# JiawangBian/SC-SfMLearner-Release

Measured on AMD Instinct MI355X. Metric: train images/sec (+ warp-loss ms/step) KITTI 256x832 RN18, higher is better.
Workload: dtype f32; 1 GPU; configs[1]: kitti 256x832, batch 12/GPU, 2 refs (seq 3), ResNet18 DispNet + ResNet18 PoseNet, ssim+mask+auto-mask, zeros padding, 1 scale; global_batch=12, parallelism=1 GPU, memory_format=contiguous (NCHW)

## Files before the change

### __graft_entry__.py

```python
import os
import sys

ROOT = os.path.dirname(os.path.abspath(__file__))
PKG = os.path.join(ROOT, "sc-sfmlearner-release_amd")
for p in (ROOT, PKG):
    if p not in sys.path:
        sys.path.insert(0, p)


def build() -> None:
    from scsfm_hip import _lib, build as hip_build
    path = hip_build.build(force=False)
    lib = _lib.CLib(path)
    assert lib._dll.scsfm_abi_version() == _lib.ABI_VERSION
    nets_path = hip_build.build_nets(force=False)
    nets = _lib.CLib(nets_path, _lib.NETS_HEADER, _lib.NETS_ABI_VERSION, "scsfm_nets_")
    eval_path = hip_build.build_eval(force=False)
    ev = _lib.CLib(eval_path, _lib.EVAL_HEADER, _lib.EVAL_ABI_VERSION, "scsfm_eval_")
    odom_path = hip_build.build_odom(force=False)
    od = _lib.CLib(odom_path, _lib.ODOM_HEADER, _lib.ODOM_ABI_VERSION, "scsfm_odom_")
    import inverse_warp
    import loss_functions
    import models
    from scsfm_hip import decoder, depth_eval, odometry
    from oracle import scsfm_oracle
    print(f"[build] {path}: {len(lib.decls)} entry points resolved")
    print(f"[build] {nets_path}: {len(nets.decls)} entry points resolved")
    print(f"[build] {eval_path}: {len(ev.decls)} entry points resolved")
    print(f"[build] {odom_path}: {len(od.decls)} entry points resolved")


def smoke() -> None:
    import torch

    import loss_functions as LF
    from oracle import scsfm_oracle as O
    from scsfm_hip import _lib, synth

    assert torch.cuda.is_available(), "smoke() needs a HIP device"
    lib = _lib.get()
    assert lib.path.endswith("libscsfm_hip.so")
    dev = torch.device("cuda:0")
    d = synth.make_batch(2, 128, 416, n_ref=2, seed=0, depth="smooth")

    def leaves(device):
        mv = lambda t: t.to(device).clone().requires_grad_(True)
        return ([mv(t) for t in d["tgt_depth"]], [[mv(t) for t in r] for r in d["ref_depths"]],
                [mv(p) for p in d["poses"]], [mv(p) for p in d["poses_inv"]])

    td, rd, ps, pi = leaves(dev)
    tgt, refs, K = d["tgt_img"].to(dev), [r.to(dev) for r in d["ref_imgs"]], d["intrinsics"].to(dev)
    photo, geom = LF.compute_photo_and_geometry_loss(tgt, refs, K, td, rd, ps, pi, 1, 1, 1, 1, "zeros")
    smooth = LF.compute_smooth_loss(td, tgt, rd, refs)
    (photo + 0.1 * smooth + 0.5 * geom).backward()
    torch.cuda.synchronize()

    td_c, rd_c, ps_c, pi_c = leaves("cpu")
    photo_c, geom_c = O.photo_and_geometry_loss(d["tgt_img"], d["ref_imgs"], d["intrinsics"], td_c, rd_c, ps_c, pi_c,
                                                1, 1, 1, 1, "zeros")
    smooth_c = O.smooth_loss(td_c, d["tgt_img"], rd_c, d["ref_imgs"])
    (photo_c + 0.1 * smooth_c + 0.5 * geom_c).backward()
    for name, a, b in (("photo", photo, photo_c), ("geom", geom, geom_c), ("smooth", smooth, smooth_c)):
        err = abs(float(a) - float(b))
        print(f"[smoke] {name}: hip {float(a):.7f} oracle {float(b):.7f} |d| {err:.2e}")
        assert err <= 1e-5, name
    pairs = [("g_tgt_depth", td[0].grad, td_c[0].grad), ("g_ref0_depth", rd[0][0].grad, rd_c[0][0].grad),
             ("g_ref1_depth", rd[1][0].grad, rd_c[1][0].grad), ("g_pose0", ps[0].grad, ps_c[0].grad),
             ("g_pose_inv1", pi[1].grad, pi_c[1].grad)]
    for name, a, b in pairs:
        scale = float(b.abs().max())
        bad = ((a.cpu() - b).abs() > 0.01 * scale).double().mean().item()
        print(f"[smoke] {name}: scale {scale:.3e} share of entries off by >1% of scale {bad:.2e}")
        assert bad <= 2e-3, name
    print("[smoke] ok")


if __name__ == "__main__":
    build()
    if "--smoke" in sys.argv:
        smoke()
```

### sc-sfmlearner-release_amd/models/resnet_encoder.py

```python
from __future__ import absolute_import, division, print_function

import numpy as np
import torch
import torch.nn as nn


def _conv3x3(cin, cout, stride=1):
    return nn.Conv2d(cin, cout, kernel_size=3, stride=stride, padding=1, bias=False)


class BasicBlock(nn.Module):
    expansion = 1

    def __init__(self, inplanes, planes, stride=1, downsample=None):
        super().__init__()
        self.conv1 = _conv3x3(inplanes, planes, stride)
        self.bn1 = nn.BatchNorm2d(planes)
        self.relu = nn.ReLU(inplace=True)
        self.conv2 = _conv3x3(planes, planes)
        self.bn2 = nn.BatchNorm2d(planes)
        self.downsample = downsample

    def forward(self, x):
        identity = x if self.downsample is None else self.downsample(x)
        out = self.relu(self.bn1(self.conv1(x)))
        out = self.bn2(self.conv2(out))
        return self.relu(out + identity)


class Bottleneck(nn.Module):
    expansion = 4

    def __init__(self, inplanes, planes, stride=1, downsample=None):
        super().__init__()
        self.conv1 = nn.Conv2d(inplanes, planes, kernel_size=1, bias=False)
        self.bn1 = nn.BatchNorm2d(planes)
        self.conv2 = _conv3x3(planes, planes, stride)
        self.bn2 = nn.BatchNorm2d(planes)
        self.conv3 = nn.Conv2d(planes, planes * 4, kernel_size=1, bias=False)
        self.bn3 = nn.BatchNorm2d(planes * 4)
        self.relu = nn.ReLU(inplace=True)
        self.downsample = downsample

    def forward(self, x):
        identity = x if self.downsample is None else self.downsample(x)
        out = self.relu(self.bn1(self.conv1(x)))
        out = self.relu(self.bn2(self.conv2(out)))
        out = self.bn3(self.conv3(out))
        return self.relu(out + identity)


class ResNet(nn.Module):

    def __init__(self, block, layers, num_classes=1000, num_input_images=1):
        super().__init__()
        self.inplanes = 64
        self.conv1 = nn.Conv2d(num_input_images * 3, 64, kernel_size=7, stride=2, padding=3, bias=False)
        self.bn1 = nn.BatchNorm2d(64)
        self.relu = nn.ReLU(inplace=True)
        self.maxpool = nn.MaxPool2d(kernel_size=3, stride=2, padding=1)
        self.layer1 = self._make_layer(block, 64, layers[0])
        self.layer2 = self._make_layer(block, 128, layers[1], stride=2)
        self.layer3 = self._make_layer(block, 256, layers[2], stride=2)
        self.layer4 = self._make_layer(block, 512, layers[3], stride=2)
        self.avgpool = nn.AdaptiveAvgPool2d((1, 1))
        self.fc = nn.Linear(512 * block.expansion, num_classes)
        for m in self.modules():
            if isinstance(m, nn.Conv2d):
                nn.init.kaiming_normal_(m.weight, mode='fan_out', nonlinearity='relu')
            elif isinstance(m, nn.BatchNorm2d):
                nn.init.constant_(m.weight, 1)
                nn.init.constant_(m.bias, 0)

    def _make_layer(self, block, planes, blocks, stride=1):
        downsample = None
        if stride != 1 or self.inplanes != planes * block.expansion:
            downsample = nn.Sequential(
                nn.Conv2d(self.inplanes, planes * block.expansion, kernel_size=1, stride=stride, bias=False),
                nn.BatchNorm2d(planes * block.expansion))
        layers = [block(self.inplanes, planes, stride, downsample)]
        self.inplanes = planes * block.expansion
        layers += [block(self.inplanes, planes) for _ in range(1, blocks)]
        return nn.Sequential(*layers)


_CFG = {18: (BasicBlock, [2, 2, 2, 2]), 50: (Bottleneck, [3, 4, 6, 3])}


def imagenet_weights_path(num_layers):
    import os
    root = os.environ.get("SCSFM_IMAGENET_WEIGHTS")
    if not root:
        return None
    path = os.path.join(root, "resnet{}.pth".format(num_layers))
    return path if os.path.exists(path) else None


class ResnetEncoder(nn.Module):

    def __init__(self, num_layers, pretrained, num_input_images=1):
        super().__init__()
        if num_layers not in _CFG:
            raise ValueError("{} is not a valid number of resnet layers".format(num_layers))
        block, layers = _CFG[num_layers]
        self.num_ch_enc = np.array([64, 64, 128, 256, 512])
        if num_layers > 34:
            self.num_ch_enc[1:] *= 4
        self.encoder = ResNet(block, layers, num_input_images=num_input_images)
        if pretrained:
            path = imagenet_weights_path(num_layers)
            if path is None:
                raise RuntimeError("ImageNet-pretrained weights are not reachable offline: set SCSFM_IMAGENET_WEIGHTS "
                                   "to a directory holding resnet{}.pth, or use --with-pretrain 0".format(num_layers))
            loaded = torch.load(path, map_location="cpu")
            loaded['conv1.weight'] = torch.cat([loaded['conv1.weight']] * num_input_images, 1) / num_input_images
            self.encoder.load_state_dict(loaded)
        for p in self.encoder.fc.parameters():
            p.requires_grad_(False)

    def forward(self, input_image):
        e = self.encoder
        f0 = e.relu(e.bn1(e.conv1(input_image)))
        f1 = e.layer1(e.maxpool(f0))
        f2 = e.layer2(f1)
        f3 = e.layer3(f2)
        f4 = e.layer4(f3)
        self.features = [f0, f1, f2, f3, f4]
        return self.features
```

### sc-sfmlearner-release_amd/scsfm_hip/_lib.py

```python
from __future__ import annotations

import ctypes
import os
import re
import threading

import torch

HERE = os.path.dirname(os.path.abspath(__file__))
HEADER = os.path.join(os.path.dirname(os.path.dirname(HERE)), "include", "scsfm_hip.h")
LIB_PATH = os.environ.get("SCSFM_HIP_LIB") or os.path.join(HERE, "libscsfm_hip.so")

ABI_VERSION = 9

_CTYPES = {"int": ctypes.c_int, "unsigned": ctypes.c_uint, "size_t": ctypes.c_size_t, "double": ctypes.c_double}
_DECL = re.compile(r"^(int|size_t)\s+(scsfm_\w+)\s*\(([^)]*)\)\s*;", re.M | re.S)


def parse_header(path=HEADER):
    text = open(path).read()
    text = re.sub(r"/\*.*?\*/", "", text, flags=re.S)
    out = {}
    for ret, name, args in _DECL.findall(text):
        argtypes = []
        args = " ".join(args.split())
        if args and args != "void":
            for a in args.split(","):
                a = a.strip()
                if "*" in a:
                    argtypes.append(ctypes.c_void_p)
                else:
                    argtypes.append(_CTYPES[a.split()[0]])
        out[name] = (_CTYPES[ret], argtypes)
    return out


class ScsfmError(RuntimeError):
    pass


class CLib:

    def __init__(self, path, header=HEADER, abi=ABI_VERSION, prefix="scsfm_"):
        self.path = path
        self._dll = ctypes.CDLL(path)
        self.decls = parse_header(header)
        self._fn = {}
        self._prefix = prefix
        for name, (ret, argtypes) in self.decls.items():
            try:
                fn = getattr(self._dll, name)
            except AttributeError as e:
                raise ScsfmError(f"{path} does not export {name} (declared in {header})") from e
            fn.restype = ret
            fn.argtypes = argtypes
            self._fn[name] = fn
        if self._fn[prefix + "abi_version"]() != abi:
            raise ScsfmError(f"{path}: ABI version mismatch")

    def source_id(self):
        buf = ctypes.create_string_buffer(64)
        self._fn[self._prefix + "source_id"](buf, 64)
        return buf.value.decode()

    def call(self, name, *args):
        rc = self._fn[name](*args)
        if rc != 0:
            kind = "rejected argument" if rc == -1 else "hipError_t"
            raise ScsfmError(f"{name} failed with status {rc} ({kind})")

    def size(self, name, *args):
        return int(self._fn[name](*args))


_lock = threading.Lock()
_lib = None


def get() -> CLib:
    global _lib
    if _lib is None:
        with _lock:
            if _lib is None:
                from . import build as _build
                own = "SCSFM_HIP_LIB" not in os.environ
                if own and _build.is_stale():
                    have = _build.binary_source_id(LIB_PATH)
                    try:
                        _build.build()
                    except Exception as e:
                        what = f"was built from other sources ({have}) than the tree's ({_build.source_id()})" if have \
                            else "is missing (or carries no source id)"
                        raise ScsfmError(f"{LIB_PATH} {what} and cannot be built here: {e}") from e
                lib = CLib(LIB_PATH)
                if own and lib.source_id() != _build.source_id():
                    raise ScsfmError(f"{LIB_PATH}: its source id {lib.source_id()} is not the tree's {_build.source_id()}")
                _lib = lib
    return _lib


NETS_HEADER = os.path.join(os.path.dirname(os.path.dirname(HERE)), "include", "scsfm_nets.h")
NETS_LIB_PATH = os.path.join(HERE, "libscsfm_nets.so")
NETS_ABI_VERSION = 1
_nets = None


def get_nets() -> CLib:
    global _nets
    if _nets is None:
        with _lock:
            if _nets is None:
                from . import build as _build
                if _build.nets_is_stale():
                    have = _build.binary_source_id(NETS_LIB_PATH)
                    try:
                        _build.build_nets()
                    except Exception as e:
                        raise ScsfmError(f"{NETS_LIB_PATH} is stale or missing ({have}) and cannot be built here: {e}") \
                            from e
                lib = CLib(NETS_LIB_PATH, NETS_HEADER, NETS_ABI_VERSION, "scsfm_nets_")
                if lib.source_id() != _build.nets_source_id():
                    raise ScsfmError(f"{NETS_LIB_PATH}: its source id {lib.source_id()} is not the tree's "
                                     f"{_build.nets_source_id()}")
                _nets = lib
    return _nets


EVAL_HEADER = os.path.join(os.path.dirname(os.path.dirname(HERE)), "include", "scsfm_eval.h")
EVAL_LIB_PATH = os.path.join(HERE, "libscsfm_eval.so")
EVAL_ABI_VERSION = 1
_eval = None


def get_eval() -> CLib:
    global _eval
    if _eval is None:
        with _lock:
            if _eval is None:
                from . import build as _build
                if _build.eval_is_stale():
                    have = _build.binary_source_id(EVAL_LIB_PATH)
                    try:
                        _build.build_eval()
                    except Exception as e:
                        raise ScsfmError(f"{EVAL_LIB_PATH} is stale or missing ({have}) and cannot be built here: {e}") \
                            from e
                lib = CLib(EVAL_LIB_PATH, EVAL_HEADER, EVAL_ABI_VERSION, "scsfm_eval_")
                if lib.source_id() != _build.eval_source_id():
                    raise ScsfmError(f"{EVAL_LIB_PATH}: its source id {lib.source_id()} is not the tree's "
                                     f"{_build.eval_source_id()}")
                _eval = lib
    return _eval


ODOM_HEADER = os.path.join(os.path.dirname(os.path.dirname(HERE)), "include", "scsfm_odom.h")
ODOM_LIB_PATH = os.path.join(HERE, "libscsfm_odom.so")
ODOM_ABI_VERSION = 1
_odom = None


def get_odom() -> CLib:
    global _odom
    if _odom is None:
        with _lock:
            if _odom is None:
                from . import build as _build
                if _build.odom_is_stale():
                    have = _build.binary_source_id(ODOM_LIB_PATH)
                    try:
                        _build.build_odom()
                    except Exception as e:
                        raise ScsfmError(f"{ODOM_LIB_PATH} is stale or missing ({have}) and cannot be built here: {e}") \
                            from e
                lib = CLib(ODOM_LIB_PATH, ODOM_HEADER, ODOM_ABI_VERSION, "scsfm_odom_")
                if lib.source_id() != _build.odom_source_id():
                    raise ScsfmError(f"{ODOM_LIB_PATH}: its source id {lib.source_id()} is not the tree's "
                                     f"{_build.odom_source_id()}")
                _odom = lib
    return _odom
```

### sc-sfmlearner-release_amd/scsfm_hip/build.py

```python
from __future__ import annotations

import contextlib
import fcntl
import glob
import hashlib
import os
import shutil
import subprocess
import sys
import tempfile

HERE = os.path.dirname(os.path.abspath(__file__))
CSRC = os.path.join(os.path.dirname(HERE), "csrc")
LIB = os.path.join(HERE, "libscsfm_hip.so")
LOCK = LIB + ".lock"
LOG = LIB + ".buildlog"
INCLUDE = os.path.join(os.path.dirname(os.path.dirname(HERE)), "include")
NETS_CSRC = os.path.join(os.path.dirname(HERE), "csrc_nets")
NETS_LIB = os.path.join(HERE, "libscsfm_nets.so")
EVAL_CSRC = os.path.join(os.path.dirname(HERE), "csrc_eval")
EVAL_LIB = os.path.join(HERE, "libscsfm_eval.so")
ODOM_CSRC = os.path.join(os.path.dirname(HERE), "csrc_odom")
ODOM_LIB = os.path.join(HERE, "libscsfm_odom.so")
ARCH = "gfx950"
FLAGS = ["-O3", "-std=c++17", "-fPIC", "-shared", f"--offload-arch={ARCH}", "-munsafe-fp-atomics",
         "-fno-gpu-rdc", "-Wall", "-Wno-unused-function",
         "-fno-slp-vectorize"]
ID_MARKER = b"scsfm-source-id:"


def sources():
    return sorted(glob.glob(os.path.join(CSRC, "*.hip")))


def deps():
    return sources() + sorted(glob.glob(os.path.join(CSRC, "*.h"))) + \
        [os.path.join(INCLUDE, "scsfm_hip.h")]


def nets_sources():
    return sorted(glob.glob(os.path.join(NETS_CSRC, "*.hip")))


def nets_deps():
    return nets_sources() + sorted(glob.glob(os.path.join(NETS_CSRC, "*.h"))) + [os.path.join(INCLUDE, "scsfm_nets.h")]


def eval_sources():
    return sorted(glob.glob(os.path.join(EVAL_CSRC, "*.hip")))


def eval_deps():
    return eval_sources() + sorted(glob.glob(os.path.join(EVAL_CSRC, "*.h"))) + [os.path.join(INCLUDE, "scsfm_eval.h")]


def odom_sources():
    return sorted(glob.glob(os.path.join(ODOM_CSRC, "*.hip")))


def odom_deps():
    return odom_sources() + sorted(glob.glob(os.path.join(ODOM_CSRC, "*.h"))) + [os.path.join(INCLUDE, "scsfm_odom.h")]


def _hash(files, extra=()):
    h = hashlib.sha256()
    for path in files:
        h.update(os.path.basename(path).encode())
        h.update(open(path, "rb").read())
    h.update(" ".join(FLAGS).encode())
    if extra:
        h.update(b"\0extra:" + " ".join(extra).encode())
    return h.hexdigest()[:16]


def source_id(extra=()):
    files = deps()
    if any("SCSFM_WITH_MARCH" in e or "variants" in e for e in extra):
        vsrc = os.path.join(os.path.dirname(os.path.dirname(HERE)), "variants", "src")
        files = files + sorted(p for p in glob.glob(os.path.join(vsrc, "*")) if os.path.isfile(p))
    return _hash(files, extra)


def nets_source_id():
    return _hash(nets_deps())


def eval_source_id():
    return _hash(eval_deps())


def odom_source_id():
    return _hash(odom_deps())


def binary_source_id(path=LIB):
    try:
        blob = open(path, "rb").read()
    except OSError:
        return None
    i = blob.find(ID_MARKER)
    if i < 0:
        return None
    j = i + len(ID_MARKER)
    return blob[j:j + 16].decode("ascii", "replace")


def is_stale():
    return binary_source_id(LIB) != source_id()


def nets_is_stale():
    return binary_source_id(NETS_LIB) != nets_source_id()


def eval_is_stale():
    return binary_source_id(EVAL_LIB) != eval_source_id()


def odom_is_stale():
    return binary_source_id(ODOM_LIB) != odom_source_id()


@contextlib.contextmanager
def _build_lock(lock=None):
    fd = os.open(lock or LOCK, os.O_CREAT | os.O_RDWR, 0o644)
    try:
        fcntl.flock(fd, fcntl.LOCK_EX)
        yield
    finally:
        try:
            fcntl.flock(fd, fcntl.LOCK_UN)
        finally:
            os.close(fd)


def build(force=False, verbose=True, extra=()):
    extra = tuple(extra)
    return _build(LIB, source_id(extra), sources(), extra, force, verbose)


def build_nets(force=False, verbose=True):
    return _build(NETS_LIB, nets_source_id(), nets_sources(), ("-I", INCLUDE), force, verbose)


def build_eval(force=False, verbose=True):
    return _build(EVAL_LIB, eval_source_id(), eval_sources(), ("-I", INCLUDE), force, verbose)


def build_odom(force=False, verbose=True):
    return _build(ODOM_LIB, odom_source_id(), odom_sources(), ("-I", INCLUDE), force, verbose)


def _build(lib, want, srcs, extra, force, verbose):
    if not force and binary_source_id(lib) == want:
        return lib
    with _build_lock(lib + ".lock"):
        if not force and binary_source_id(lib) == want:
            return lib
        hipcc = shutil.which("hipcc") or "/opt/rocm/bin/hipcc"
        name = os.path.basename(lib)
        if not os.path.exists(hipcc):
            raise RuntimeError(f"hipcc not found: {name} cannot be built on this machine")
        fd, tmp = tempfile.mkstemp(prefix=name[:-len(".so")] + ".", suffix=f".{os.getpid()}.tmp", dir=HERE)
        os.close(fd)
        try:
            cmd = [hipcc, *FLAGS, f'-DSCSFM_SOURCE_ID="{want}"', *extra, "-o", tmp, *srcs]
            if verbose:
                print("[scsfm_hip.build]", " ".join(cmd), flush=True)
            subprocess.run(cmd, check=True)
            os.chmod(tmp, 0o755)
            os.replace(tmp, lib)
            with open(lib + ".buildlog", "a") as f:
                f.write(f"{want} {os.getpid()}\n")
        finally:
            if os.path.exists(tmp):
                os.unlink(tmp)
    return lib


if __name__ == "__main__":
    build(force="--force" in sys.argv)
    build_nets(force="--force" in sys.argv)
    build_eval(force="--force" in sys.argv)
    build_odom(force="--force" in sys.argv)
    print(LIB)
    print(NETS_LIB)
    print(EVAL_LIB)
    print(ODOM_LIB)
```

Measured before the change: 125.2 images/s.

## Add fused HIP BatchNorm+ReLU+residual and maxpool kernels for ResNet encoder

Adds a new HIP library with training-mode BatchNorm kernels that fuse the normalisation with an optional ReLU and residual add. Statistics are reduced in double precision across split blocks per channel. It also adds a max-pool forward that stores a compact uint8 argmax, and a matching backward. Autograd wrappers expose these as `bn_act` and `max_pool`, with build and ABI plumbing for a separate shared library. The aim is to cut the separate elementwise kernel launches and memory passes of the stock BN, ReLU and add ops in ResNet18, at the cost of custom code that must match PyTorch BN semantics.

```diff
diff --git a/__graft_entry__.py b/__graft_entry__.py
--- a/__graft_entry__.py
+++ b/__graft_entry__.py
@@ -19,15 +19,18 @@
     ev = _lib.CLib(eval_path, _lib.EVAL_HEADER, _lib.EVAL_ABI_VERSION, "scsfm_eval_")
     odom_path = hip_build.build_odom(force=False)
     od = _lib.CLib(odom_path, _lib.ODOM_HEADER, _lib.ODOM_ABI_VERSION, "scsfm_odom_")
+    enc_path = hip_build.build_enc(force=False)
+    enc = _lib.CLib(enc_path, _lib.ENC_HEADER, _lib.ENC_ABI_VERSION, "scsfm_enc_")
     import inverse_warp
     import loss_functions
     import models
-    from scsfm_hip import decoder, depth_eval, odometry
+    from scsfm_hip import decoder, depth_eval, encoder, odometry
     from oracle import scsfm_oracle
     print(f"[build] {path}: {len(lib.decls)} entry points resolved")
     print(f"[build] {nets_path}: {len(nets.decls)} entry points resolved")
     print(f"[build] {eval_path}: {len(ev.decls)} entry points resolved")
     print(f"[build] {odom_path}: {len(od.decls)} entry points resolved")
+    print(f"[build] {enc_path}: {len(enc.decls)} entry points resolved")
 
 
 def smoke() -> None:
diff --git a/include/scsfm_enc.h b/include/scsfm_enc.h
--- /dev/null
+++ b/include/scsfm_enc.h
@@ -0,0 +1,32 @@
+#ifndef SCSFM_ENC_H_
+#define SCSFM_ENC_H_
+
+#include <stddef.h>
+
+#ifdef __cplusplus
+extern "C" {
+#endif
+
+int scsfm_enc_abi_version(void);
+int scsfm_enc_source_id(char* buf, size_t n);
+
+size_t scsfm_enc_bn_workspace_bytes(int B, int C, int H, int W);
+
+int scsfm_enc_bn_fwd_f32(int B, int C, int H, int W, int mode, double eps, double momentum, const float* x,
+                         const float* identity, const float* gamma, const float* beta, float* y, float* stat,
+                         float* running_mean, float* running_var, long long* num_batches_tracked, void* ws,
+                         size_t ws_bytes, void* stream);
+
+int scsfm_enc_bn_bwd_f32(int B, int C, int H, int W, int mode, const float* g, const float* x, const float* y,
+                         const float* gamma, const float* beta, const float* stat, float* dx, float* d_identity,
+                         float* dgamma, float* dbeta, void* ws, size_t ws_bytes, void* stream);
+
+int scsfm_enc_maxpool_fwd_f32(int B, int C, int H, int W, const float* x, float* out, unsigned char* arg, void* stream);
+int scsfm_enc_maxpool_bwd_f32(int B, int C, int H, int W, const float* g, const unsigned char* arg, float* dx,
+                              void* stream);
+
+#ifdef __cplusplus
+}
+#endif
+
+#endif
diff --git a/sc-sfmlearner-release_amd/csrc_enc/scsfm_encoder.hip b/sc-sfmlearner-release_amd/csrc_enc/scsfm_encoder.hip
--- /dev/null
+++ b/sc-sfmlearner-release_amd/csrc_enc/scsfm_encoder.hip
@@ -0,0 +1,446 @@
+#include <hip/hip_runtime.h>
+
+#include "scsfm_enc.h"
+
+namespace scsfm_enc {
+
+constexpr int kWave = 64;
+constexpr int kThreads = 256;
+constexpr int kWaves = kThreads / kWave;
+constexpr int kMaxSplit = 64;
+constexpr int kTargetBlocks = 2048;
+constexpr int kUnroll = 4;
+constexpr int kUnrollEw = 2;
+
+template <int V>
+struct Pack {
+  float v[V];
+};
+template <int V>
+__device__ inline Pack<V> load(const float* __restrict__ p);
+template <>
+__device__ inline Pack<1> load<1>(const float* __restrict__ p) {
+  return {{p[0]}};
+}
+template <>
+__device__ inline Pack<4> load<4>(const float* __restrict__ p) {
+  const float4 t = *reinterpret_cast<const float4*>(p);
+  return {{t.x, t.y, t.z, t.w}};
+}
+__device__ inline void store(float* __restrict__ p, const Pack<1>& a) { p[0] = a.v[0]; }
+__device__ inline void store(float* __restrict__ p, const Pack<4>& a) {
+  float4 t;
+  t.x = a.v[0]; t.y = a.v[1]; t.z = a.v[2]; t.w = a.v[3];
+  *reinterpret_cast<float4*>(p) = t;
+}
+
+__device__ inline int imin(int a, int b) { return a < b ? a : b; }
+__device__ inline int imax(int a, int b) { return a > b ? a : b; }
+
+struct Geo {
+  int C, HW, per, units;
+};
+template <int V>
+__device__ inline int offset_of(const Geo& g, int c, int u) {
+  const int b = u / g.per;
+  return (b * g.C + c) * g.HW + (u - b * g.per) * V;
+}
+__device__ inline void range(const Geo& g, int& u0, int& u1) {
+  const long long S = gridDim.y, s = blockIdx.y;
+  u0 = (int)(g.units * s / S);
+  u1 = (int)(g.units * (s + 1) / S);
+}
+
+__device__ inline double wave_sum(double v) {
+#pragma unroll
+  for (int d = kWave / 2; d > 0; d >>= 1) v += __shfl_down(v, d);
+  return v;
+}
+
+__device__ inline void block_sum_to(double a, double b, double* __restrict__ part) {
+  __shared__ double red[2 * kWaves];
+  a = wave_sum(a);
+  b = wave_sum(b);
+  const int lane = threadIdx.x & (kWave - 1), wave = threadIdx.x >> 6;
+  if (lane == 0) {
+    red[2 * wave] = a;
+    red[2 * wave + 1] = b;
+  }
+  __syncthreads();
+  if (threadIdx.x == 0) {
+    double ta = red[0], tb = red[1];
+#pragma unroll
+    for (int w = 1; w < kWaves; ++w) {
+      ta += red[2 * w];
+      tb += red[2 * w + 1];
+    }
+    double* dst = part + 2 * ((size_t)blockIdx.x * gridDim.y + blockIdx.y);
+    dst[0] = ta;
+    dst[1] = tb;
+  }
+}
+
+__device__ inline void channel_totals(const double* __restrict__ part, double& a, double& b) {
+  const int lane = threadIdx.x & (kWave - 1), S = gridDim.y;
+  const double* src = part + 2 * ((size_t)blockIdx.x * S + imin(lane, S - 1));
+  a = wave_sum(lane < S ? src[0] : 0.0);
+  b = wave_sum(lane < S ? src[1] : 0.0);
+}
+
+__device__ inline float relu(float v) { return v > 0.f ? v : (v != v ? v : 0.f); }
+__device__ inline float xhat_of(float x, float mean, float mean_lo, float invstd) { return ((x - mean) - mean_lo) * invstd; }
+__device__ inline float bn_value(float xh, float gamma, float beta) { return fmaf(xh, gamma, beta); }
+
+template <int V>
+__global__ __launch_bounds__(kThreads) void bn_stats_kernel(Geo geo, const float* __restrict__ x,
+                                                             double* __restrict__ part) {
+  const int c = blockIdx.x;
+  int u0, u1;
+  range(geo, u0, u1);
+  double s = 0.0, q = 0.0;
+  for (int u = u0 + (int)threadIdx.x; u < u1; u += kUnroll * kThreads) {
+    Pack<V> p[kUnroll];
+#pragma unroll
+    for (int j = 0; j < kUnroll; ++j) p[j] = load<V>(x + offset_of<V>(geo, c, imin(u + j * kThreads, u1 - 1)));
+#pragma unroll
+    for (int j = 0; j < kUnroll; ++j) {
+      if (u + j * kThreads < u1) {
+#pragma unroll
+        for (int k = 0; k < V; ++k) {
+          const double d = (double)p[j].v[k];
+          s += d;
+          q = fma(d, d, q);
+        }
+      }
+    }
+  }
+  block_sum_to(s, q, part);
+}
+
+template <int V, int MODE>
+__global__ __launch_bounds__(kThreads) void bn_apply_fwd_kernel(
+    Geo geo, double inv_n, double unbias, double eps, double momentum, const float* __restrict__ x,
+    const float* __restrict__ identity, const float* __restrict__ gamma, const float* __restrict__ beta,
+    const double* __restrict__ part, float* __restrict__ y, float* __restrict__ stat, float* __restrict__ running_mean,
+    float* __restrict__ running_var, long long* __restrict__ num_batches_tracked) {
+  __shared__ float sh[3];
+  const int c = blockIdx.x;
+  if (threadIdx.x < kWave) {
+    double s, q;
+    channel_totals(part, s, q);
+    if (threadIdx.x == 0) {
+      const double m = s * inv_n;
+      double var = q * inv_n - m * m;
+      if (var < 0.0) var = 0.0;
+      const float mf = (float)m, lo = (float)(m - (double)mf), is = (float)(1.0 / sqrt(var + eps));
+      sh[0] = mf;
+      sh[1] = is;
+      sh[2] = lo;
+      if (blockIdx.y == 0) {
+        stat[c] = mf;
+        stat[geo.C + c] = is;
+        stat[2 * geo.C + c] = lo;
+        running_mean[c] = (float)((1.0 - momentum) * (double)running_mean[c] + momentum * m);
+        running_var[c] = (float)((1.0 - momentum) * (double)running_var[c] + momentum * var * unbias);
+        if (c == 0) num_batches_tracked[0] += 1;
+      }
+    }
+  }
+  __syncthreads();
+  const float mean = sh[0], invstd = sh[1], mean_lo = sh[2], ga = gamma[c], be = beta[c];
+  int u0, u1;
+  range(geo, u0, u1);
+  for (int u = u0 + (int)threadIdx.x; u < u1; u += kUnrollEw * kThreads) {
+    Pack<V> p[kUnrollEw], r[kUnrollEw];
+    int off[kUnrollEw];
+#pragma unroll
+    for (int j = 0; j < kUnrollEw; ++j) {
+      off[j] = offset_of<V>(geo, c, imin(u + j * kThreads, u1 - 1));
+      p[j] = load<V>(x + off[j]);
+      if (MODE == 2) r[j] = load<V>(identity + off[j]);
+    }
+#pragma unroll
+    for (int j = 0; j < kUnrollEw; ++j) {
+      if (u + j * kThreads < u1) {
+        Pack<V> o;
+#pragma unroll
+        for (int k = 0; k < V; ++k) {
+          float v = bn_value(xhat_of(p[j].v[k], mean, mean_lo, invstd), ga, be);
+          if (MODE == 2) v += r[j].v[k];
+          o.v[k] = MODE == 0 ? v : relu(v);
+        }
+        store(y + off[j], o);
+      }
+    }
+  }
+}
+
+template <int MODE>
+__device__ inline float masked(float g, float xh, float ga, float be, float yv) {
+  if (MODE == 1) return bn_value(xh, ga, be) <= 0.f ? 0.f : g;
+  if (MODE == 2) return yv <= 0.f ? 0.f : g;
+  return g;
+}
+
+template <int V, int MODE>
+__global__ __launch_bounds__(kThreads) void bn_bwd_reduce_kernel(Geo geo, const float* __restrict__ g,
+                                                                  const float* __restrict__ x,
+                                                                  const float* __restrict__ y,
+                                                                  const float* __restrict__ gamma,
+                                                                  const float* __restrict__ beta,
+                                                                  const float* __restrict__ stat,
+                                                                  double* __restrict__ part) {
+  const int c = blockIdx.x;
+  const float mean = stat[c], invstd = stat[geo.C + c], mean_lo = stat[2 * geo.C + c], ga = gamma[c], be = beta[c];
+  int u0, u1;
+  range(geo, u0, u1);
+  double sb = 0.0, sg = 0.0;
+  for (int u = u0 + (int)threadIdx.x; u < u1; u += kUnrollEw * kThreads) {
+    Pack<V> pg[kUnrollEw], px[kUnrollEw], py[kUnrollEw];
+#pragma unroll
+    for (int j = 0; j < kUnrollEw; ++j) {
+      const int off = offset_of<V>(geo, c, imin(u + j * kThreads, u1 - 1));
+      pg[j] = load<V>(g + off);
+      px[j] = load<V>(x + off);
+      if (MODE == 2) py[j] = load<V>(y + off);
+    }
+#pragma unroll
+    for (int j = 0; j < kUnrollEw; ++j) {
+      if (u + j * kThreads < u1) {
+#pragma unroll
+        for (int k = 0; k < V; ++k) {
+          const float xh = xhat_of(px[j].v[k], mean, mean_lo, invstd);
+          const double gm = (double)masked<MODE>(pg[j].v[k], xh, ga, be, MODE == 2 ? py[j].v[k] : 0.f);
+          sb += gm;
+          sg = fma(gm, (double)xh, sg);
+        }
+      }
+    }
+  }
+  block_sum_to(sb, sg, part);
+}
+
+template <int V, int MODE>
+__global__ __launch_bounds__(kThreads) void bn_bwd_dx_kernel(Geo geo, double inv_n, const float* __restrict__ g,
+                                                              const float* __restrict__ x, const float* __restrict__ y,
+                                                              const float* __restrict__ gamma,
+                                                              const float* __restrict__ beta,
+                                                              const float* __restrict__ stat,
+                                                              const double* __restrict__ part, float* __restrict__ dx,
+                                                              float* __restrict__ d_identity, float* __restrict__ dgamma,
+                                                              float* __restrict__ dbeta) {
+  __shared__ float sh[2];
+  const int c = blockIdx.x;
+  if (threadIdx.x < kWave) {
+    double sb, sg;
+    channel_totals(part, sb, sg);
+    if (threadIdx.x == 0) {
+      sh[0] = (float)(sb * inv_n);
+      sh[1] = (float)(sg * inv_n);
+      if (blockIdx.y == 0) {
+        dbeta[c] = (float)sb;
+        dgamma[c] = (float)sg;
+      }
+    }
+  }
+  __syncthreads();
+  const float mean = stat[c], invstd = stat[geo.C + c], mean_lo = stat[2 * geo.C + c], ga = gamma[c], be = beta[c];
+  const float mb = sh[0], mg = sh[1], k1 = ga * invstd;
+  int u0, u1;
+  range(geo, u0, u1);
+  for (int u = u0 + (int)threadIdx.x; u < u1; u += kUnrollEw * kThreads) {
+    Pack<V> pg[kUnrollEw], px[kUnrollEw], py[kUnrollEw];
+    int off[kUnrollEw];
+#pragma unroll
+    for (int j = 0; j < kUnrollEw; ++j) {
+      off[j] = offset_of<V>(geo, c, imin(u + j * kThreads, u1 - 1));
+      pg[j] = load<V>(g + off[j]);
+      px[j] = load<V>(x + off[j]);
+      if (MODE == 2) py[j] = load<V>(y + off[j]);
+    }
+#pragma unroll
+    for (int j = 0; j < kUnrollEw; ++j) {
+      if (u + j * kThreads < u1) {
+        Pack<V> o, m;
+#pragma unroll
+        for (int k = 0; k < V; ++k) {
+          const float xh = xhat_of(px[j].v[k], mean, mean_lo, invstd);
+          m.v[k] = masked<MODE>(pg[j].v[k], xh, ga, be, MODE == 2 ? py[j].v[k] : 0.f);
+          o.v[k] = ((m.v[k] - mb) - xh * mg) * k1;
+        }
+        store(dx + off[j], o);
+        if (MODE == 2) store(d_identity + off[j], m);
+      }
+    }
+  }
+}
+
+static __global__ __launch_bounds__(kThreads) void maxpool_fwd_kernel(int total, int H, int W, int PH, int PW,
+                                                                const float* __restrict__ x, float* __restrict__ out,
+                                                                unsigned char* __restrict__ arg) {
+  const int i = blockIdx.x * kThreads + threadIdx.x;
+  if (i >= total) return;
+  const int t = i / PW, pw = i - t * PW, plane = t / PH, ph = t - plane * PH;
+  const int hs = 2 * ph - 1, ws = 2 * pw - 1;
+  const int h0 = imax(hs, 0), h1 = imin(hs + 3, H), w0 = imax(ws, 0), w1 = imin(ws + 3, W);
+  const float* src = x + (size_t)plane * H * W;
+  float best = -INFINITY;
+  int at = (h0 - hs) * 3 + (w0 - ws);
+  for (int h = h0; h < h1; ++h)
+    for (int w = w0; w < w1; ++w) {
+      const float v = src[h * W + w];
+      if (v > best || v != v) {
+        best = v;
+        at = (h - hs) * 3 + (w - ws);
+      }
+    }
+  out[i] = best;
+  arg[i] = (unsigned char)at;
+}
+
+static __global__ __launch_bounds__(kThreads) void maxpool_bwd_kernel(int total, int H, int W, int PH, int PW,
+                                                                const float* __restrict__ g,
+                                                                const unsigned char* __restrict__ arg,
+                                                                float* __restrict__ dx) {
+  const int i = blockIdx.x * kThreads + threadIdx.x;
+  if (i >= total) return;
+  const int t = i / W, w = i - t * W, plane = t / H, h = t - plane * H;
+  const int ph0 = h / 2, ph1 = imin((h + 1) / 2, PH - 1), pw0 = w / 2, pw1 = imin((w + 1) / 2, PW - 1);
+  const int base = plane * PH * PW;
+  float acc = 0.f;
+  for (int ph = ph0; ph <= ph1; ++ph)
+    for (int pw = pw0; pw <= pw1; ++pw) {
+      const int o = base + ph * PW + pw;
+      if ((int)arg[o] == (h - 2 * ph + 1) * 3 + (w - 2 * pw + 1)) acc += g[o];
+    }
+  dx[i] = acc;
+}
+
+inline int ceil_div(long long a, long long b) { return (int)((a + b - 1) / b); }
+
+inline bool bn_shape_ok(int B, int C, int H, int W) {
+  if (B <= 0 || C <= 0 || H <= 0 || W <= 0) return false;
+  const long long n = (long long)B * H * W;
+  return n >= 2 && n * C < (1ll << 31);
+}
+
+inline bool aligned16(const void* p) { return ((size_t)p & 15) == 0; }
+
+inline Geo geometry(int B, int C, int H, int W, bool vec) {
+  const int HW = H * W, per = vec ? HW / 4 : HW;
+  return {C, HW, per, B * per};
+}
+
+inline int splits(int C, int units) {
+  int S = ceil_div(kTargetBlocks, C);
+  const int most = ceil_div(units, kThreads);
+  if (S > most) S = most;
+  if (S > kMaxSplit) S = kMaxSplit;
+  return S < 1 ? 1 : S;
+}
+
+inline int launch_status() { return (int)hipGetLastError(); }
+
+}
+
+using namespace scsfm_enc;
+
+#define SCSFM_ENC_BY_MODE(KERNEL, V, ...)                                                            \
+  do {                                                                                               \
+    if (mode == 0) hipLaunchKernelGGL((KERNEL<V, 0>), grid, block, 0, (hipStream_t)stream, __VA_ARGS__);      \
+    else if (mode == 1) hipLaunchKernelGGL((KERNEL<V, 1>), grid, block, 0, (hipStream_t)stream, __VA_ARGS__); \
+    else hipLaunchKernelGGL((KERNEL<V, 2>), grid, block, 0, (hipStream_t)stream, __VA_ARGS__);                \
+  } while (0)
+
+extern "C" {
+
+int scsfm_enc_abi_version(void) { return 1; }
+
+#ifndef SCSFM_SOURCE_ID
+#define SCSFM_SOURCE_ID "unknown"
+#endif
+static const char g_source_tag[] __attribute__((used)) = "scsfm-source-id:" SCSFM_SOURCE_ID;
+int scsfm_enc_source_id(char* buf, size_t n) {
+  const volatile char* id = g_source_tag + 16;
+  if (!buf || n == 0) return -1;
+  size_t i = 0;
+  for (; i + 1 < n && id[i]; ++i) buf[i] = id[i];
+  buf[i] = 0;
+  return 0;
+}
+
+size_t scsfm_enc_bn_workspace_bytes(int B, int C, int H, int W) {
+  if (!bn_shape_ok(B, C, H, W)) return 0;
+  return (size_t)C * kMaxSplit * 2 * sizeof(double);
+}
+
+int scsfm_enc_bn_fwd_f32(int B, int C, int H, int W, int mode, double eps, double momentum, const float* x,
+                         const float* identity, const float* gamma, const float* beta, float* y, float* stat,
+                         float* running_mean, float* running_var, long long* num_batches_tracked, void* ws,
+                         size_t ws_bytes, void* stream) {
+  if (!bn_shape_ok(B, C, H, W) || mode < 0 || mode > 2 || !(eps >= 0.0) || !(momentum >= 0.0 && momentum <= 1.0) ||
+      !x || (mode == 2 && !identity) || !gamma || !beta || !y || !stat || !running_mean || !running_var ||
+      !num_batches_tracked || !ws || ((size_t)ws & 7) || ws_bytes < scsfm_enc_bn_workspace_bytes(B, C, H, W))
+    return -1;
+  (void)hipGetLastError();
+  const bool vec = (H * W) % 4 == 0 && aligned16(x) && aligned16(y) && (mode != 2 || aligned16(identity));
+  const Geo geo = geometry(B, C, H, W, vec);
+  const dim3 grid(C, splits(C, geo.units)), block(kThreads);
+  const double n = (double)B * H * W, inv_n = 1.0 / n, unbias = n / (n - 1.0);
+  double* part = (double*)ws;
+  if (vec) {
+    hipLaunchKernelGGL(bn_stats_kernel<4>, grid, block, 0, (hipStream_t)stream, geo, x, part);
+    SCSFM_ENC_BY_MODE(bn_apply_fwd_kernel, 4, geo, inv_n, unbias, eps, momentum, x, identity, gamma, beta, part, y,
+                      stat, running_mean, running_var, num_batches_tracked);
+  } else {
+    hipLaunchKernelGGL(bn_stats_kernel<1>, grid, block, 0, (hipStream_t)stream, geo, x, part);
+    SCSFM_ENC_BY_MODE(bn_apply_fwd_kernel, 1, geo, inv_n, unbias, eps, momentum, x, identity, gamma, beta, part, y,
+                      stat, running_mean, running_var, num_batches_tracked);
+  }
+  return launch_status();
+}
+
+int scsfm_enc_bn_bwd_f32(int B, int C, int H, int W, int mode, const float* g, const float* x, const float* y,
+                         const float* gamma, const float* beta, const float* stat, float* dx, float* d_identity,
+                         float* dgamma, float* dbeta, void* ws, size_t ws_bytes, void* stream) {
+  if (!bn_shape_ok(B, C, H, W) || mode < 0 || mode > 2 || !g || !x || (mode == 2 && (!y || !d_identity)) || !gamma ||
+      !beta || !stat || !dx || !dgamma || !dbeta || !ws || ((size_t)ws & 7) ||
+      ws_bytes < scsfm_enc_bn_workspace_bytes(B, C, H, W))
+    return -1;
+  (void)hipGetLastError();
+  const bool vec = (H * W) % 4 == 0 && aligned16(g) && aligned16(x) && aligned16(dx) &&
+                   (mode != 2 || (aligned16(y) && aligned16(d_identity)));
+  const Geo geo = geometry(B, C, H, W, vec);
+  const dim3 grid(C, splits(C, geo.units)), block(kThreads);
+  const double inv_n = 1.0 / ((double)B * H * W);
+  double* part = (double*)ws;
+  if (vec) {
+    SCSFM_ENC_BY_MODE(bn_bwd_reduce_kernel, 4, geo, g, x, y, gamma, beta, stat, part);
+    SCSFM_ENC_BY_MODE(bn_bwd_dx_kernel, 4, geo, inv_n, g, x, y, gamma, beta, stat, part, dx, d_identity, dgamma, dbeta);
+  } else {
+    SCSFM_ENC_BY_MODE(bn_bwd_reduce_kernel, 1, geo, g, x, y, gamma, beta, stat, part);
+    SCSFM_ENC_BY_MODE(bn_bwd_dx_kernel, 1, geo, inv_n, g, x, y, gamma, beta, stat, part, dx, d_identity, dgamma, dbeta);
+  }
+  return launch_status();
+}
+
+int scsfm_enc_maxpool_fwd_f32(int B, int C, int H, int W, const float* x, float* out, unsigned char* arg, void* stream) {
+  if (B <= 0 || C <= 0 || H <= 0 || W <= 0 || !x || !out || !arg || (long long)B * C * H * W >= (1ll << 31)) return -1;
+  (void)hipGetLastError();
+  const int PH = (H - 1) / 2 + 1, PW = (W - 1) / 2 + 1, total = B * C * PH * PW;
+  hipLaunchKernelGGL(maxpool_fwd_kernel, dim3(ceil_div(total, kThreads)), dim3(kThreads), 0, (hipStream_t)stream, total,
+                     H, W, PH, PW, x, out, arg);
+  return launch_status();
+}
+
+int scsfm_enc_maxpool_bwd_f32(int B, int C, int H, int W, const float* g, const unsigned char* arg, float* dx,
+                              void* stream) {
+  if (B <= 0 || C <= 0 || H <= 0 || W <= 0 || !g || !arg || !dx || (long long)B * C * H * W >= (1ll << 31)) return -1;
+  (void)hipGetLastError();
+  const int PH = (H - 1) / 2 + 1, PW = (W - 1) / 2 + 1, total = B * C * H * W;
+  hipLaunchKernelGGL(maxpool_bwd_kernel, dim3(ceil_div(total, kThreads)), dim3(kThreads), 0, (hipStream_t)stream, total,
+                     H, W, PH, PW, g, arg, dx);
+  return launch_status();
+}
+
+}
diff --git a/sc-sfmlearner-release_amd/models/resnet_encoder.py b/sc-sfmlearner-release_amd/models/resnet_encoder.py
--- a/sc-sfmlearner-release_amd/models/resnet_encoder.py
+++ b/sc-sfmlearner-release_amd/models/resnet_encoder.py
@@ -3,6 +3,34 @@
 import numpy as np
 import torch
 import torch.nn as nn
+
+
+_encoder_ops = None
+
+
+def _E():
+    global _encoder_ops
+    if _encoder_ops is None:
+        from scsfm_hip import encoder
+        _encoder_ops = encoder
+    return _encoder_ops
+
+
+def _fused_applies(x, *bns):
+    return x.is_cuda and _E().applies(x, *bns)
+
+
+def _bn_act(x, bn, act, identity=None):
+    if _fused_applies(x, bn) and (identity is None or _fused_applies(identity)):
+        return _E().bn_act(x, bn, identity, relu=act is not None)
+    out = bn(x)
+    if identity is not None:
+        out = out + identity
+    return out if act is None else act(out)
+
+
+def _downsample(ds, x):
+    return _bn_act(ds[0](x), ds[1], None)
 
 
 def _conv3x3(cin, cout, stride=1):
@@ -22,6 +50,11 @@
         self.downsample = downsample
 
     def forward(self, x):
+        identity = x if self.downsample is None else _downsample(self.downsample, x)
+        out = _bn_act(self.conv1(x), self.bn1, self.relu)
+        return _bn_act(self.conv2(out), self.bn2, self.relu, identity)
+
+    def forward_reference(self, x):
         identity = x if self.downsample is None else self.downsample(x)
         out = self.relu(self.bn1(self.conv1(x)))
         out = self.bn2(self.conv2(out))
@@ -43,6 +76,12 @@
         self.downsample = downsample
 
     def forward(self, x):
+        identity = x if self.downsample is None else _downsample(self.downsample, x)
+        out = _bn_act(self.conv1(x), self.bn1, self.relu)
+        out = _bn_act(self.conv2(out), self.bn2, self.relu)
+        return _bn_act(self.conv3(out), self.bn3, self.relu, identity)
+
+    def forward_reference(self, x):
         identity = x if self.downsample is None else self.downsample(x)
         out = self.relu(self.bn1(self.conv1(x)))
         out = self.relu(self.bn2(self.conv2(out)))
@@ -120,10 +159,26 @@
 
     def forward(self, input_image):
         e = self.encoder
-        f0 = e.relu(e.bn1(e.conv1(input_image)))
-        f1 = e.layer1(e.maxpool(f0))
+        f0 = _bn_act(e.conv1(input_image), e.bn1, e.relu)
+        f1 = e.layer1(self._maxpool(f0))
         f2 = e.layer2(f1)
         f3 = e.layer3(f2)
         f4 = e.layer4(f3)
         self.features = [f0, f1, f2, f3, f4]
         return self.features
+
+    def _maxpool(self, f0):
+        e = self.encoder
+        if f0.is_cuda and e.training and _E().pool_applies(f0):
+            return _E().max_pool(f0)
+        return e.maxpool(f0)
+
+    def forward_reference(self, input_image):
+        e = self.encoder
+        f0 = e.relu(e.bn1(e.conv1(input_image)))
+        feats, x = [f0], e.maxpool(f0)
+        for layer in (e.layer1, e.layer2, e.layer3, e.layer4):
+            for block in layer:
+                x = block.forward_reference(x)
+            feats.append(x)
+        return feats
diff --git a/sc-sfmlearner-release_amd/scsfm_hip/_lib.py b/sc-sfmlearner-release_amd/scsfm_hip/_lib.py
--- a/sc-sfmlearner-release_amd/scsfm_hip/_lib.py
+++ b/sc-sfmlearner-release_amd/scsfm_hip/_lib.py
@@ -178,3 +178,30 @@
                                      f"{_build.odom_source_id()}")
                 _odom = lib
     return _odom
+
+
+ENC_HEADER = os.path.join(os.path.dirname(os.path.dirname(HERE)), "include", "scsfm_enc.h")
+ENC_LIB_PATH = os.path.join(HERE, "libscsfm_enc.so")
+ENC_ABI_VERSION = 1
+_enc = None
+
+
+def get_enc() -> CLib:
+    global _enc
+    if _enc is None:
+        with _lock:
+            if _enc is None:
+                from . import build as _build
+                if _build.enc_is_stale():
+                    have = _build.binary_source_id(ENC_LIB_PATH)
+                    try:
+                        _build.build_enc()
+                    except Exception as e:
+                        raise ScsfmError(f"{ENC_LIB_PATH} is stale or missing ({have}) and cannot be built here: {e}") \
+                            from e
+                lib = CLib(ENC_LIB_PATH, ENC_HEADER, ENC_ABI_VERSION, "scsfm_enc_")
+                if lib.source_id() != _build.enc_source_id():
+                    raise ScsfmError(f"{ENC_LIB_PATH}: its source id {lib.source_id()} is not the tree's "
+                                     f"{_build.enc_source_id()}")
+                _enc = lib
+    return _enc
diff --git a/sc-sfmlearner-release_amd/scsfm_hip/build.py b/sc-sfmlearner-release_amd/scsfm_hip/build.py
--- a/sc-sfmlearner-release_amd/scsfm_hip/build.py
+++ b/sc-sfmlearner-release_amd/scsfm_hip/build.py
@@ -22,6 +22,8 @@
 EVAL_LIB = os.path.join(HERE, "libscsfm_eval.so")
 ODOM_CSRC = os.path.join(os.path.dirname(HERE), "csrc_odom")
 ODOM_LIB = os.path.join(HERE, "libscsfm_odom.so")
+ENC_CSRC = os.path.join(os.path.dirname(HERE), "csrc_enc")
+ENC_LIB = os.path.join(HERE, "libscsfm_enc.so")
 ARCH = "gfx950"
 FLAGS = ["-O3", "-std=c++17", "-fPIC", "-shared", f"--offload-arch={ARCH}", "-munsafe-fp-atomics",
          "-fno-gpu-rdc", "-Wall", "-Wno-unused-function",
@@ -60,6 +62,14 @@
 
 def odom_deps():
     return odom_sources() + sorted(glob.glob(os.path.join(ODOM_CSRC, "*.h"))) + [os.path.join(INCLUDE, "scsfm_odom.h")]
+
+
+def enc_sources():
+    return sorted(glob.glob(os.path.join(ENC_CSRC, "*.hip")))
+
+
+def enc_deps():
+    return enc_sources() + sorted(glob.glob(os.path.join(ENC_CSRC, "*.h"))) + [os.path.join(INCLUDE, "scsfm_enc.h")]
 
 
 def _hash(files, extra=()):
@@ -91,6 +101,10 @@
 
 def odom_source_id():
     return _hash(odom_deps())
+
+
+def enc_source_id():
+    return _hash(enc_deps())
 
 
 def binary_source_id(path=LIB):
@@ -119,6 +133,10 @@
 
 def odom_is_stale():
     return binary_source_id(ODOM_LIB) != odom_source_id()
+
+
+def enc_is_stale():
+    return binary_source_id(ENC_LIB) != enc_source_id()
 
 
 @contextlib.contextmanager
@@ -149,6 +167,10 @@
 
 def build_odom(force=False, verbose=True):
     return _build(ODOM_LIB, odom_source_id(), odom_sources(), ("-I", INCLUDE), force, verbose)
+
+
+def build_enc(force=False, verbose=True):
+    return _build(ENC_LIB, enc_source_id(), enc_sources(), ("-I", INCLUDE), force, verbose)
 
 
 def _build(lib, want, srcs, extra, force, verbose):
@@ -183,7 +205,9 @@
     build_nets(force="--force" in sys.argv)
     build_eval(force="--force" in sys.argv)
     build_odom(force="--force" in sys.argv)
+    build_enc(force="--force" in sys.argv)
     print(LIB)
     print(NETS_LIB)
     print(EVAL_LIB)
     print(ODOM_LIB)
+    print(ENC_LIB)
diff --git a/sc-sfmlearner-release_amd/scsfm_hip/encoder.py b/sc-sfmlearner-release_amd/scsfm_hip/encoder.py
--- /dev/null
+++ b/sc-sfmlearner-release_amd/scsfm_hip/encoder.py
@@ -0,0 +1,115 @@
+from __future__ import annotations
+
+import torch
+from torch.autograd.function import once_differentiable
+
+from . import _lib
+from .capi import _stream
+
+
+def _plain(t):
+    return t.is_cuda and t.dtype == torch.float32 and t.is_contiguous()
+
+
+def applies(x, *bns):
+    if not (torch.is_tensor(x) and x.dim() == 4 and _plain(x) and x.numel() < 2 ** 31 and
+            x.shape[0] * x.shape[2] * x.shape[3] >= 2):
+        return False
+    for bn in bns:
+        if not (bn.training and bn.affine and bn.track_running_stats and bn.momentum is not None):
+            return False
+        if not all(_plain(t) for t in (bn.weight, bn.bias, bn.running_mean, bn.running_var)):
+            return False
+        if not (bn.num_batches_tracked.is_cuda and bn.num_batches_tracked.dtype == torch.int64):
+            return False
+    return True
+
+
+def pool_applies(x):
+    return torch.is_tensor(x) and x.dim() == 4 and _plain(x) and 0 < x.numel() < 2 ** 31
+
+
+def _workspace(lib, x):
+    B, C, H, W = x.shape
+    n = lib.size("scsfm_enc_bn_workspace_bytes", B, C, H, W)
+    return torch.empty(n // 8, dtype=torch.float64, device=x.device), n
+
+
+class _BnAct(torch.autograd.Function):
+    @staticmethod
+    def forward(ctx, x, identity, weight, bias, bn, mode):
+        lib = _lib.get_enc()
+        B, C, H, W = x.shape
+        if identity is not None and (identity.shape != x.shape or not _plain(identity)):
+            raise ValueError(f"bn_act: identity {tuple(identity.shape)} does not match x {tuple(x.shape)}")
+        y = torch.empty_like(x)
+        stat = torch.empty((3, C), dtype=torch.float32, device=x.device)
+        ws, n = _workspace(lib, x)
+        lib.call("scsfm_enc_bn_fwd_f32", B, C, H, W, mode, float(bn.eps), float(bn.momentum), x.data_ptr(),
+                 0 if identity is None else identity.data_ptr(), weight.data_ptr(), bias.data_ptr(), y.data_ptr(),
+                 stat.data_ptr(), bn.running_mean.data_ptr(), bn.running_var.data_ptr(),
+                 bn.num_batches_tracked.data_ptr(), ws.data_ptr(), n, _stream(x))
+        ctx.mode = mode
+        ctx.save_for_backward(x, weight, bias, stat, *((y,) if mode == 2 else ()))
+        return y
+
+    @staticmethod
+    @once_differentiable
+    def backward(ctx, g):
+        lib = _lib.get_enc()
+        g = g.contiguous()
+        x, weight, bias, stat = ctx.saved_tensors[:4]
+        y = ctx.saved_tensors[4] if ctx.mode == 2 else None
+        B, C, H, W = x.shape
+        dx = torch.empty_like(x)
+        d_id = torch.empty_like(x) if ctx.mode == 2 else None
+        dgamma = torch.empty(C, dtype=torch.float32, device=x.device)
+        dbeta = torch.empty(C, dtype=torch.float32, device=x.device)
+        ws, n = _workspace(lib, x)
+        lib.call("scsfm_enc_bn_bwd_f32", B, C, H, W, ctx.mode, g.data_ptr(), x.data_ptr(),
+                 0 if y is None else y.data_ptr(), weight.data_ptr(), bias.data_ptr(), stat.data_ptr(), dx.data_ptr(),
+                 0 if d_id is None else d_id.data_ptr(), dgamma.data_ptr(), dbeta.data_ptr(), ws.data_ptr(), n,
+                 _stream(x))
+        return dx, d_id, dgamma, dbeta, None, None
+
+
+class _MaxPool(torch.autograd.Function):
+    @staticmethod
+    def forward(ctx, x):
+        B, C, H, W = x.shape
+        PH, PW = (H - 1) // 2 + 1, (W - 1) // 2 + 1
+        out = torch.empty((B, C, PH, PW), dtype=x.dtype, device=x.device)
+        arg = torch.empty((B, C, PH, PW), dtype=torch.uint8, device=x.device)
+        _lib.get_enc().call("scsfm_enc_maxpool_fwd_f32", B, C, H, W, x.data_ptr(), out.data_ptr(), arg.data_ptr(),
+                            _stream(x))
+        ctx.save_for_backward(arg)
+        ctx.shape = (B, C, H, W)
+        return out
+
+    @staticmethod
+    @once_differentiable
+    def backward(ctx, g):
+        g = g.contiguous()
+        (arg,) = ctx.saved_tensors
+        B, C, H, W = ctx.shape
+        dx = torch.empty((B, C, H, W), dtype=g.dtype, device=g.device)
+        _lib.get_enc().call("scsfm_enc_maxpool_bwd_f32", B, C, H, W, g.data_ptr(), arg.data_ptr(), dx.data_ptr(),
+                            _stream(g))
+        return dx
+
+
+def bn_act(x, bn, identity=None, relu=True):
+    if not applies(x, bn):
+        raise ValueError("scsfm_hip.encoder.bn_act: CUDA fp32 contiguous NCHW input and a training-mode affine "
+                         f"BatchNorm2d with running statistics only (got {x.device} {x.dtype} {tuple(x.shape)})")
+    if identity is not None and not relu:
+        raise ValueError("bn_act: the residual form ends in a ReLU")
+    mode = 2 if identity is not None else (1 if relu else 0)
+    return _BnAct.apply(x, identity, bn.weight, bn.bias, bn, mode)
+
+
+def max_pool(x):
+    if not pool_applies(x):
+        raise ValueError("scsfm_hip.encoder.max_pool: CUDA fp32 contiguous NCHW tensors only "
+                         f"(got {x.device} {x.dtype} {tuple(x.shape)})")
+    return _MaxPool.apply(x)
```

New measurement: 137.4 images/s (median of 6 runs). +9.8%, better.
